# isaac-chandler/cuda-raytracer

Measured on AMD Instinct MI355X. Metric: Mrays/s (live ray segments/s, teapot), higher is better.
Workload: dtype f32

## Files before the change

### cuda-raytracer_amd/csrc/rt_render.hip

```cpp
#include "rt_common.h"

#include <algorithm>
#include <chrono>
#include <cstdio>
#include <cstdlib>
#include <cstring>
#include <string>
#include <thread>
#include <vector>

#include <rccl/rccl.h>

#pragma clang fp contract(off)

int rtamd_render_multi(const rt_scene *scene, const rt_opts *opts, float *fb_out, rt_stats *stats);

using namespace rtamd;

namespace {

#ifndef RT_INFLIGHT
#define RT_INFLIGHT 20
#endif
#ifndef RT_TRACE_OCC
// ... 50 lines not shown
    static FastDiv of(uint32_t d) {
        FastDiv f;
        if (d > 1) {
            f.l = 32 - __builtin_clz(d - 1);
            f.m = (uint32_t)((((uint64_t)1 << (31 + f.l)) + d - 1) / d);
        }
        return f;
    }
    __device__ __forceinline__ uint32_t div(uint32_t n) const { return l == 0 ? n : (__umulhi(n, m) >> (l - 1)); }
};

struct SlotMap {
    FastDiv by_stripe;
    uint32_t skip, base;
    static SlotMap identity() { return SlotMap{FastDiv::of(0x7fffffffu), 0u, 0u}; }
    static SlotMap of(uint32_t stripe, int count, int index) {
        return SlotMap{FastDiv::of(stripe), (uint32_t)(count - 1) * stripe, (uint32_t)index * stripe};
    }
    __device__ __forceinline__ uint32_t ray(uint32_t s) const { return s + by_stripe.div(s) * skip + base; }
};

template <int FIRST>
__device__ __forceinline__ uint32_t first_ray(const SlotMap &m, uint32_t slot) {
    return FIRST == 2 ? m.ray(slot) : slot;
}

struct PassArgs {
    int rtc;
    uint32_t gen_seed_term;
    FastDiv by_rtc, by_width;
    SlotMap map;
};

__device__ __forceinline__ V3 primary_dir(const DevScene &S, int i, const PassArgs &pa) {
    Rng rng = pcg_seed((uint32_t)i * 0x85810BEAu + pa.gen_seed_term);
    uint32_t z;
    asm volatile("v_mov_b32 %0, 0" : "=v"(z));
    rng.inc += z;
    const uint32_t pixel = pa.by_rtc.div((uint32_t)i);
    const uint32_t yy = pa.by_width.div(pixel);
    const int x = (int)(pixel - yy * (uint32_t)S.width), y = (int)yy;
    const float xc = (x + random01(rng)) * S.inv_w;
    const float yc = (y + random01(rng)) * S.inv_h;
    return normalise(S.tl + xc * S.sr - yc * S.su);
}

#ifndef RT_FUSED_MAX_TRIS
#define RT_FUSED_MAX_TRIS 4096
#endif
#ifndef RT_SORT_GRID
#define RT_SORT_GRID 0
#endif

template <bool SORTED, bool COUNT, int FIRST>
__global__ __launch_bounds__(kBlock) RT_TRACE_ATTR void trace_kernel(DevScene S, PassArgs pa, const float4 *__restrict__ geo,
                                                       const uint32_t *__restrict__ live_count,
                                                       uint32_t *__restrict__ queue, float2 *__restrict__ hits,
                                                       uint32_t *__restrict__ overflow, Counters *__restrict__ ctr,
                                                       unsigned long long *__restrict__ tspan) {
    __shared__ uint2 stack[(kStackLds + 1) * kBlock];
    const unsigned long long t_start = wall_clock64();
    uint2 *col = stack + threadIdx.x;
    const uint32_t lanes = gridDim.x * kBlock, gl = blockIdx.x * kBlock + threadIdx.x;
    const uint32_t dist_half = lanes * (kStackMax - kStackLds);
    const uint32_t L = __builtin_amdgcn_readfirstlane(*live_count);
    const uint32_t waves = gridDim.x * (kBlock / 64);
    const uint32_t chunk = min((uint32_t)kChunkMax, max((uint32_t)kChunkMin, (L / (4 * waves) + 63) & ~63u));
    uint32_t shard = blockIdx.x % kQueues, tried = 0;
    uint32_t q_next = 0, q_end = 0;
    bool exhausted = false;
    int slot = -1;
    V3 o{0, 0, 0}, d{0, 0, 0};
    float ix = 0, iy = 0, iz = 0, closest = 0;
    bool finite_inv = true;
    bool wave_nonfinite = false;
    int index = -1, sp = 0;
    uint32_t ref = 0;
    int ti = 0, te = 0;
    unsigned pn = 0, iv = 0, tt = 0, nlive = 0;
#ifdef RT_PROFILE
    unsigned long long prof[14] = {0, 0, 0, 0, 0, 0, 0, 0, 0, 0, 0, 0, 0, 0};
#endif
    auto node_step = [&](float4 a, float4 b, float4 c, uint2 kids) -> bool {
        if (COUNT) iv++;
        float t0, t1;
        bool h0, h1;
        slab_pair(a, b, c, o, ix, iy, iz, closest, h0, h1, t0, t1);
        if (__builtin_expect(wave_nonfinite, 0)) {
            float u0, u1;
            const bool g0 = slab(a.x, a.z, b.x, b.z, c.x, c.z, o, ix, iy, iz, closest, u0);
            const bool g1 = slab(a.y, a.w, b.y, b.w, c.y, c.w, o, ix, iy, iz, closest, u1);
            if (!finite_inv) { h0 = g0; h1 = g1; t0 = u0; t1 = u1; }
        }
        const bool both = h0 && h1, any = h0 || h1;
        const bool sel1 = h1 && (!h0 || t0 < t1);
        const uint32_t next_ref = sel1 ? kids.y : kids.x, near_ref = sel1 ? kids.x : kids.y;
        const float next_t = sel1 ? t1 : t0, near_t = sel1 ? t0 : t1;
        col[min(sp, kStackLds) * kBlock] = make_uint2(near_ref, __float_as_uint(near_t));
        if (__builtin_expect(both && sp >= kStackLds, 0)) {
            overflow[(sp - kStackLds) * lanes + gl] = near_ref;
            overflow[dist_half + (sp - kStackLds) * lanes + gl] = __float_as_uint(near_t);
        }
        if (both) sp++;
        ref = any ? next_ref : ref;
        const bool descend = any && !(next_t >= closest);
        bool need = !descend;
        if (descend) {
            if (COUNT) pn++;
            if (ref & kLeaf) {
                leaf_range(S, ref, ti, te);
                need = ti == te;
            }
        }
        return need;
    };
    auto pop_loop = [&](bool need) {
        while (need) {
            PROF(10, 1);
            const bool empty = sp == 0;
            sp = empty ? 0 : sp - 1;
            uint2 e = col[min(sp, kStackLds) * kBlock];
            asm volatile("" : "+v"(e.x), "+v"(e.y));
            if (__builtin_expect(__ballot(sp >= kStackLds) != 0, 0)) {
                if (sp >= kStackLds) {
                    e.x = overflow[(sp - kStackLds) * lanes + gl];
                    e.y = overflow[dist_half + (sp - kStackLds) * lanes + gl];
                }
            }
            const bool take = !empty && !(__uint_as_float(e.y) >= closest);
            slot = empty ? -2 - slot : slot;
            ref = take ? e.x : ref;
            if (COUNT) pn += take ? 1u : 0u;
            const bool leaf = take && (ref & kLeaf);
            if (__builtin_expect(leaf && (ref & kBigLeaf), 0)) {
                leaf_range(S, ref, ti, te);
            } else {
                ti = leaf ? (int)(ref & 0xFFFFFFu) : ti;
                te = leaf ? ti + (int)((ref >> 24) & 0x3Fu) : te;
            }
            need = !empty && (!take || (leaf && ti == te));
        }
    };
    const bool root_internal = !(S.root_ref & kLeaf);
    float4 ra{0, 0, 0, 0}, rb{0, 0, 0, 0}, rc{0, 0, 0, 0};
    uint2 rk{0, 0};
    if (root_internal) {
        const float4 *rr = S.nodes + (size_t)S.root_ref * 4;
        const float4 x0 = rr[0], x1 = rr[1], x2 = rr[2];
        const uint2 k = *reinterpret_cast<const uint2 *>(rr + 3);
#define RT_U(v) __int_as_float(__builtin_amdgcn_readfirstlane(__float_as_int(v)))
        ra = make_float4(RT_U(x0.x), RT_U(x0.y), RT_U(x0.z), RT_U(x0.w));
        rb = make_float4(RT_U(x1.x), RT_U(x1.y), RT_U(x1.z), RT_U(x1.w));
        rc = make_float4(RT_U(x2.x), RT_U(x2.y), RT_U(x2.z), RT_U(x2.w));
#undef RT_U
        rk = make_uint2(__builtin_amdgcn_readfirstlane(k.x), __builtin_amdgcn_readfirstlane(k.y));
    }
    while (true) {
        unsigned long long idle = __ballot(slot < 0);
        if (!exhausted && __popcll(idle) >= (FIRST ? kRefillFirst : kRefill)) {
            PROF(6, 1);
            if (slot <= -2) {
                hits[-2 - slot] = make_float2(closest, __int_as_float(index));
                slot = -1;
            }
            bool fresh = false;
            while (idle && !exhausted) {
                if (q_next >= q_end) {
                    const uint32_t seg_lo = (uint32_t)(((uint64_t)L * shard) / kQueues);
                    const uint32_t seg_hi = (uint32_t)(((uint64_t)L * (shard + 1)) / kQueues);
                    uint32_t c = 0;
                    if (lane_id() == 0) c = atomicAdd(queue + shard * kQueueStride, chunk);
                    c = __builtin_amdgcn_readfirstlane(__shfl(c, 0)) + seg_lo;
                    if (c >= seg_hi) {
                        shard = (shard + 1) % kQueues;
                        if (++tried == kQueues) exhausted = true;
                        continue;
                    }
                    q_next = c;
                    q_end = min(c + chunk, seg_hi);
                }
                const uint32_t avail = q_end - q_next;
                const uint32_t r = rank_below(idle);
                const bool take = slot < 0 && r < avail;
                const unsigned long long took = __ballot(take);
                if (take) { slot = (int)(q_next + r); fresh = true; }
                q_next += (uint32_t)__popcll(took);
                idle &= ~took;
            }
            if (fresh) {
                {
                    nlive++;
                    if (FIRST) {
                        o = S.cam;
                        d = primary_dir(S, (int)first_ray<FIRST>(pa.map, (uint32_t)slot), pa);
                    } else {
                        const float4 *rp = geo + (size_t)slot * 2;
                        const float4 r0 = rp[0];
                        const float2 r1 = *reinterpret_cast<const float2 *>(rp + 1);
                        o = v3(r0.x, r0.y, r0.z);
                        d = v3(r0.w, r1.x, r1.y);
                    }
                    ix = 1 / d.x; iy = 1 / d.y; iz = 1 / d.z;
                    finite_inv = __builtin_isfinite(ix) && __builtin_isfinite(iy) && __builtin_isfinite(iz);

                    closest = 1e30f;
                    index = -1;
                    for (int i = 0; i < S.sphere_count; i++) {
                        const float4 sph = S.spheres[i];
                        float t;
                        if (ray_sphere(o, d, v3(sph.x, sph.y, sph.z), sph.w, closest, t)) { closest = t; index = i; }
                    }
                    ref = S.root_ref;
                    sp = 0;
                    if (COUNT) pn++;
                    ti = te = 0;
                    if (ref & kLeaf) {
                        leaf_range(S, ref, ti, te);
                        if (ti == te) {
                            hits[slot] = make_float2(closest, __int_as_float(index));
                            slot = -1;
                        }
                    }
                }
            }
            wave_nonfinite = __ballot(slot >= 0 && !finite_inv) != 0;
            if (root_internal && __ballot(fresh && slot >= 0)) {
                bool need = false;
                if (fresh && slot >= 0) need = node_step(ra, rb, rc, rk);
                pop_loop(need);
            }
        }
        if (!__ballot(slot >= 0)) {
            if (exhausted) break;
            PROF(7, 1);
            continue;
        }
#ifdef RT_PROFILE
        {
            const unsigned long long act = __ballot(slot >= 0), lf = __ballot(slot >= 0 && ti < te);
            PROF(0, 1); PROF(1, __popcll(act)); PROF(2, __popcll(lf));
            PROF(3, lf != 0); PROF(4, (act & ~lf) != 0);
            const bool mixed = lf != 0 && (act & ~lf) != 0;
            PROF(8, mixed);
            if (mixed) PROF(9, min(__popcll(lf), __popcll(act & ~lf)));
            const uintptr_t ra = slot >= 0 ? (uintptr_t)(ti < te ? S.tris + (size_t)ti * 3 : S.nodes + (size_t)ref * 4) : 0;
            const int first = __builtin_ctzll(act);
            const uintptr_t r0 = ((uintptr_t)__shfl((unsigned)(ra >> 32), first) << 32) | __shfl((unsigned)ra, first);
            const unsigned long long same = __ballot(slot >= 0 && ra == r0);
            PROF(12, same == act);
            PROF(13, 4 * __popcll(same) >= 3 * __popcll(act));
        }
#endif
        if (slot < 0) continue;
        bool need = false;
        const bool in_leaf = ti < te;
        const float4 *rec = in_leaf ? S.tris + (size_t)ti * 3 : S.nodes + (size_t)ref * 4;
        const float4 a = rec[0], b = rec[1], c = rec[2];
        uint2 kids = make_uint2(0, 0);
        if (!in_leaf) kids = *reinterpret_cast<const uint2 *>(rec + 3);
        if (in_leaf) {
            const float4 q0 = a, q1 = b;
            const float q2 = c.x;
            if (COUNT) tt++;
            float t;
            const bool hit =
                ray_triangle_flat(o, d, v3(q0.x, q0.y, q0.z), v3(q0.w, q1.x, q1.y), v3(q1.z, q1.w, q2), closest, t);
            closest = hit ? t : closest;
            index = hit ? S.sphere_count + ti : index;
            need = ++ti == te;
        } else {
            need = node_step(a, b, c, kids);
        }
#ifdef RT_PROFILE
        if (__ballot(need)) PROF(5, 1);
#endif
        pop_loop(need);
    }
    if (slot <= -2) hits[-2 - slot] = make_float2(closest, __int_as_float(index));
    Counters *cs = ctr + ((blockIdx.x * (kBlock / 64) + (threadIdx.x >> 6)) & (kCtrSlots - 1));
    const unsigned long long nl = wave_sum(nlive);
    if (COUNT) {
        const unsigned long long a = wave_sum(pn), b = wave_sum(iv), t = wave_sum(tt);
        if (lane_id() == 0) {
            atomicAdd(&cs->pn, a);
            atomicAdd(&cs->iv, b);
            atomicAdd(&cs->tt, t);
            atomicAdd(&cs->st, nl * (unsigned long long)S.sphere_count);
        }
    }
    if (lane_id() == 0 && nl) atomicAdd(&cs->live, nl);
    if (tspan) {
        __syncthreads();
        if (threadIdx.x == 0) {
            atomicMin(&tspan[blockIdx.x % kSpanSlots], t_start);
            atomicMax(&tspan[kSpanSlots + blockIdx.x % kSpanSlots], (unsigned long long)wall_clock64());
        }
    }
#ifdef RT_PROFILE
    prof[11] = wave_sum((unsigned)prof[10]);
    if (lane_id() == 0)
        for (int i = 0; i < 14; i++)
            if (i != 10) atomicAdd(&g_prof[FIRST ? 0 : 1][i], prof[i]);
#endif
}

struct Shaded {
    V3 no, nd, T;
    V3 C;
    uint32_t ray;
    int kind;
    bool acc_holds;
};
struct ShadeIn {
    float2 h;
    uint32_t ray, seed;
    bool acc_holds;
    float4 r0, r1;
    float tz;
};
template <bool SORTED, int FIRST, bool INLINE>
__device__ __forceinline__ ShadeIn shade_in(const PassArgs &pa, int slot, const float4 *__restrict__ geo,
                                            const float *__restrict__ tz, const uint32_t *__restrict__ rid,
                                            const float2 *__restrict__ hits, const uint32_t *__restrict__ seed_of) {
    ShadeIn in{};
    const uint32_t ray0 = first_ray<FIRST>(pa.map, (uint32_t)slot);
    const uint32_t rv = FIRST ? (FIRST == 2 ? ray0 : (uint32_t)slot) : rid[slot];
    in.ray = rv & ~kAccFlag;
    in.acc_holds = (rv & kAccFlag) != 0;
    in.seed = (!FIRST && seed_of) ? seed_of[slot] : (SORTED || FIRST) ? (FIRST == 2 ? ray0 : (uint32_t)slot) : in.ray;
    if (!INLINE) in.h = hits[slot];
    if (!FIRST) {
        in.r0 = geo[(size_t)slot * 2];
        in.r1 = geo[(size_t)slot * 2 + 1];
        in.tz = tz[slot];
    }
// ... 590 lines not shown
}
__global__ __launch_bounds__(kBlock) void add4_kernel(float *__restrict__ img, const float *__restrict__ add, int n) {
    const int i = blockIdx.x * kBlock + threadIdx.x;
    const int n4 = n >> 2;
    if (i < n4) {
        float4 a = reinterpret_cast<float4 *>(img)[i];
        const float4 b = reinterpret_cast<const float4 *>(add)[i];
        a.x = a.x + b.x; a.y = a.y + b.y; a.z = a.z + b.z; a.w = a.w + b.w;
        reinterpret_cast<float4 *>(img)[i] = a;
    }
    if (i < (n & 3)) img[(n4 << 2) + i] = img[(n4 << 2) + i] + add[(n4 << 2) + i];
}

__attribute__((constructor(101))) void rtamd_default_hw_queues() {
    setenv("GPU_MAX_HW_QUEUES", "24", 0);
}
int queues_granted() {
    const char *q = std::getenv("GPU_MAX_HW_QUEUES");
    const int n = q ? std::atoi(q) : 0;
    return n > 0 ? n : 4;
}

}

int rtamd::trace_closest_blocks_per_cu(int &per_cu) {
    HIPCHK(hipOccupancyMaxActiveBlocksPerMultiprocessor(&per_cu, trace_kernel<false, false, 0>, kBlock, 0));
    return RT_OK;
}
void rtamd::launch_trace_closest(bool count, int grid, hipStream_t s, const DevScene &ds, const float4 *geo,
                                 const uint32_t *live, uint32_t *queue, float2 *hits, uint32_t *overflow, Counters *ctr) {
    const PassArgs pa{1, 0u, FastDiv::of(1), FastDiv::of((uint32_t)ds.width), SlotMap::identity()};
    if (count)
        hipLaunchKernelGGL((trace_kernel<false, true, 0>), dim3(grid), dim3(kBlock), 0, s, ds, pa, geo, live, queue, hits,
                           overflow, ctr, nullptr);
    else
        hipLaunchKernelGGL((trace_kernel<false, false, 0>), dim3(grid), dim3(kBlock), 0, s, ds, pa, geo, live, queue, hits,
                           overflow, ctr, nullptr);
}

struct InitTimer {
    std::chrono::high_resolution_clock::time_point t = std::chrono::high_resolution_clock::now();
    std::string out;
    bool on = std::getenv("RTAMD_TIMING") != nullptr;
    void mark(const char *what) {
        if (!on) return;
        const auto now = std::chrono::high_resolution_clock::now();
        char buf[96];
        std::snprintf(buf, sizeof(buf), " %s %.1f ms,", what, std::chrono::duration<double, std::milli>(now - t).count());
        out += buf;
        t = now;
    }
    void report() const { if (on) std::fprintf(stderr, "rt_renderer init:%s\n", out.c_str()); }
};

struct PassCtx {
    hipStream_t stream = nullptr;
    DevBuf<float4> geo[2], acc;
    DevBuf<float> tz[2];
    DevBuf<uint32_t> rid[2], sort_counts, sort_offsets, sort_totals, live, queue, overflow;
    DevBuf<uint8_t> bkt;
    DevBuf<float2> hits;
    DevBuf<uint32_t> home_of;
    DevBuf<float> psum;
    DevBuf<uint32_t> gslot[2], newpos, glive;
    DevBuf<uint8_t> gbytes, lbytes;
    uint32_t *lg_host = nullptr;
    hipEvent_t lg_ready = nullptr;
    int t_p = 0, t_k = 0, t_b = -1, t_rtc = 0, t_rem = 0, t_n = 0, t_cur = 0, t_tiles_g = 0;
    uint64_t t_lg = 0;
    hipEvent_t fb_done = nullptr;
// ... 5 lines not shown
        if (lg_host) (void)hipHostFree(lg_host);
        if (lg_ready) (void)hipEventDestroy(lg_ready);
        for (auto e : events) (void)hipEventDestroy(e);
        if (fb_done) (void)hipEventDestroy(fb_done);
        if (done) (void)hipEventDestroy(done);
        if (stream) (void)hipStreamDestroy(stream);
    }
    int open() {
        if (stream) return RT_OK;
        HIPCHK(hipStreamCreateWithFlags(&stream, hipStreamNonBlocking));
        HIPCHK(hipEventCreateWithFlags(&fb_done, hipEventDisableTiming));
        HIPCHK(hipEventCreateWithFlags(&done, hipEventDisableTiming));
        return RT_OK;
    }
    hipEvent_t event() {
        if (ev == events.size()) {
            hipEvent_t e;
            if (hipEventCreate(&e) != hipSuccess) return nullptr;
            events.push_back(e);
        }
        return events[ev++];
    }
};

struct rt_renderer {
    bool sort = true, counters = false;
    int tile_count = 1, tile_index = 0, tile_rows = 8;
    bool pass_events = true;
    bool fused = false;
    bool inline_hits = false;
    int fused_upto = -1;
    bool home = false;
    uint32_t home_base = 0;
    int width = 0, height = 0, spp = 0, bounces = 0;
    SceneDev scene;
    DevBuf<float> fb;
    DevBuf<unsigned long long> tspans;
    int wall_khz = 0;
    std::vector<double> launch_ms;
    std::vector<uint32_t> launch_live;
    bool shade_hist = !std::getenv("RTAMD_SHADE_HIST") || std::atoi(std::getenv("RTAMD_SHADE_HIST")) != 0;
    int stagger_us = std::getenv("RTAMD_STAGGER_US") ? std::max(0, std::min(20000, std::atoi(std::getenv("RTAMD_STAGGER_US"))))
                                                    : kStaggerUs;
    int short_stagger_us = std::getenv("RTAMD_STAGGER_SHORT_US")
                               ? std::max(0, std::min(20000, std::atoi(std::getenv("RTAMD_STAGGER_SHORT_US")))) : kStaggerShortUs;
    PassCtx ctx[kInflight];
    int pass_hint = 0;
    int inflight_limit = 0;
    int trace_blocks = 0;
    int trace_blocks_max = 0;
    int nctx = 1;
    int inflight_cap = kInflight;
    hipEvent_t t_begin = nullptr, t_end = nullptr;

    ~rt_renderer() {
        (void)hipSetDevice(scene.device);
        if (run_pending && t_end) (void)hipEventSynchronize(t_end);
        for (hipEvent_t e : pass_done) (void)hipEventDestroy(e);
        if (xcomm) {
            (void)hipSetDevice(scene.device);
            if (failed) (void)ncclCommAbort(static_cast<ncclComm_t>(xcomm));
            for (auto &c : ctx)
                if (c.stream) (void)hipStreamSynchronize(c.stream);
            if (!failed) (void)ncclCommDestroy(static_cast<ncclComm_t>(xcomm));
        }
        if (xhost) (void)hipHostFree(xhost);
// ... 40 lines not shown
        if (tsort()) {
            fused = false;
            fused_upto = -1;
            inline_hits = false;
        }
        width = sc->width;
        height = sc->height;
        spp = sc->ray_count;
        bounces = sc->bounces;
        InitTimer tm;
        HIPCHK(hipSetDevice(o->device));
        tm.mark("hipSetDevice");
        if (int rc0 = ctx[0].open()) return rc0;
        tm.mark("first stream");
        HIPCHK(hipEventCreate(&t_begin));
        HIPCHK(hipEventCreate(&t_end));
        hipStream_t s0 = stream();
        int rc;
        if ((rc = scene.init(sc, o->device, s0))) return rc;
        const int64_t pixels = (int64_t)width * height;
        const int64_t max_rays = pixels * std::min(20, std::max(1, spp));
        if (max_rays > 0x7fffffff / 3) return rtamd::fail(RT_E_INVALID, "image too large for 32-bit ray indices");
        if ((rc = fb.alloc((size_t)pixels * 3))) return rc;
        int per_cu = 0;
        tm.mark("scene upload");
        HIPCHK(hipOccupancyMaxActiveBlocksPerMultiprocessor(&per_cu, trace_kernel<true, false, false>, kBlock, 0));
        tm.mark("occupancy query");
        trace_blocks_max = std::max(1, scene.cus * std::max(1, per_cu));
        trace_blocks = trace_blocks_max;
        const int tiles = tile_stride(max_rays);
        home = sort && !tiled() && bounces >= 2 && (fused || fused_upto >= 0);
        if (const char *e = std::getenv("RTAMD_HOME")) home = home && std::atoi(e) != 0;
        home_base = (uint32_t)max_rays;
        const size_t ctx_bytes = (size_t)max_rays * (2 * (32 + 4 + 4) + 16 + 1 + 8 + (tsort() ? 2 * 4 + 4 + 2 : 0) +
                                                     (home ? 16 + 4 : 0)) +
                                 (size_t)trace_blocks_max * kBlock * 8 * (kStackMax - kStackLds) + ((size_t)1 << 20);
        size_t mem_free = 0, mem_total = 0;
        HIPCHK(hipMemGetInfo(&mem_free, &mem_total));
        size_t cap = kInflight;
        if (inflight_limit > 0) cap = std::min<size_t>(cap, (size_t)inflight_limit);
        if (const char *e = std::getenv("RTAMD_INFLIGHT")) cap = std::min<size_t>(cap, (size_t)std::max(1, std::atoi(e)));
        cap = std::min<size_t>(cap, (size_t)queues_granted());
        inflight_cap = (int)cap;
        if (pass_hint > 0) cap = std::min<size_t>(cap, (size_t)pass_hint);
        nctx = (int)std::min<size_t>({cap, (size_t)std::max(1, pass_count()),
                                                    std::max<size_t>(1, mem_free / 2 / ctx_bytes)});
        if (tsort() && (size_t)nctx < std::min<size_t>(cap, (size_t)std::max(1, pass_count())))
            return rtamd::fail(RT_E_OOM, "pixel tiles with sort on: device memory holds only " + std::to_string(nctx) +
                                             " passes in flight; set RTAMD_INFLIGHT to the same lower value on every owner");
        const int inflight = nctx;
        for (int k = 0; k < inflight; k++) {
            PassCtx &c = ctx[k];
            if ((rc = c.open())) return rc;
            for (int q = 0; q < 2; q++) {
                if ((rc = c.geo[q].alloc((size_t)max_rays * 2))) return rc;
                if ((rc = c.tz[q].alloc((size_t)max_rays))) return rc;
                if ((rc = c.rid[q].alloc((size_t)max_rays))) return rc;
            }
            if ((rc = c.bkt.alloc((size_t)max_rays))) return rc;
            if ((rc = c.acc.alloc((size_t)max_rays * (home ? 2 : 1)))) return rc;
            if (home && (rc = c.home_of.alloc((size_t)max_rays))) return rc;
            if ((rc = c.sort_counts.alloc((size_t)kBuckets * tiles))) return rc;
            if ((rc = c.sort_offsets.alloc((size_t)kBuckets * tiles))) return rc;
            if ((rc = c.sort_totals.alloc(kBuckets))) return rc;
            if ((rc = c.live.alloc((size_t)bounces + 1))) return rc;
            if ((rc = c.queue.alloc((size_t)(bounces + 1) * kQueues * kQueueStride))) return rc;
// ... 31 lines not shown
        const int sgrid = std::min(grid, scene.cus * RT_SHADE_BPC);
        const int sort_grid = std::max(1, std::min(max_tiles(n), RT_SORT_GRID > 0 ? RT_SORT_GRID : scene.cus * 8));
        hipStream_t st = c.stream;
        int cur = 0;
        if (n == 0) {
            for (int k = 0; pass_events && k < 3 * bounces + 2 * (bounces - 1); k++) {
                hipEvent_t e = c.event();
                if (!e) return rtamd::fail(RT_E_HIP, "hipEventCreate failed");
                HIPCHK(hipEventRecord(e, st));
            }
            HIPCHK(hipMemsetAsync(sums, 0, (size_t)pixels * 3 * sizeof(float), st));
            return RT_OK;
        }
        hipLaunchKernelGGL(fill_live_kernel, dim3(1), dim3(256), 0, st, c.live.p, (uint32_t)n, bounces + 1, c.queue.p, tspan);
        const uint32_t stripe_px = (uint32_t)(tile_rows * width);
        const SlotMap pix = tiled() ? SlotMap::of(stripe_px, tile_count, tile_index) : SlotMap::identity();
        const SlotMap map = tiled() ? SlotMap::of(stripe_px * (uint32_t)rtc, tile_count, tile_index) : SlotMap::identity();
        const PassArgs pa{rtc, 709579u * (uint32_t)remaining, FastDiv::of((uint32_t)rtc), FastDiv::of((uint32_t)width),
                          map};
        for (int b = 0; b < bounces; b++) {
            const uint32_t seed_term = 279220567u * (uint32_t)(remaining * 20 + b);
            hipEvent_t e0 = nullptr, em = nullptr, e1 = nullptr;
            if (pass_events) {
                e0 = c.event(); em = c.event(); e1 = c.event();
                if (!e0 || !em || !e1) return rtamd::fail(RT_E_HIP, "hipEventCreate failed");
                HIPCHK(hipEventRecord(e0, st));
            }
            const uint32_t *lv = c.live.p + b;
            uint32_t *q = c.queue.p + (size_t)b * kQueues * kQueueStride;
            const bool last = b + 1 == bounces;
            uint32_t *hist = shade_hist && !last ? c.sort_counts.p : nullptr;
#define RT_PROCESS3(SORTED, COUNT, FIRST)                                                                         \
    do {                                                                                                         \
        if (!inline_hits)                                                                                        \
            hipLaunchKernelGGL((trace_kernel<SORTED, COUNT, FIRST>), dim3(tgrid), dim3(kBlock), 0, st, scene.ds, pa, \
                               c.geo[cur].p, lv, q, c.hits.p, c.overflow.p, scene.ctr.p,                         \
                               tspan ? tspan + kSpanWords * b : nullptr);                                        \
        if (em) HIPCHK(hipEventRecord(em, st));                                                                  \
        if (inline_hits)                                                                                         \
            hipLaunchKernelGGL((shade_kernel<SORTED, COUNT, FIRST, true, true>), dim3(sgrid), dim3(kBlock), 0, st,\
                               scene.ds, pa, c.geo[cur].p, c.tz[cur].p, c.rid[cur].p, c.acc.p, c.bkt.p, lv, c.hits.p, \
                               seed_term, (int)last, scene.ctr.p, nullptr, hist, tiles, (int)(home && b == 0));  \
        else if (fused || b <= fused_upto)                                                                       \
            hipLaunchKernelGGL((shade_kernel<SORTED, COUNT, FIRST, true, false>), dim3(sgrid), dim3(kBlock), 0, \
                               st, scene.ds, pa, c.geo[cur].p, c.tz[cur].p, c.rid[cur].p, c.acc.p, c.bkt.p, lv, c.hits.p, \
                               seed_term, (int)last, scene.ctr.p, nullptr, hist, tiles, (int)(home && b == 0));  \
        else                                                                                                     \
            hipLaunchKernelGGL((shade_kernel<SORTED, COUNT, FIRST, false, false>), dim3(sgrid), dim3(kBlock), 0, \
                               st, scene.ds, pa, c.geo[cur].p, c.tz[cur].p, c.rid[cur].p, c.acc.p, c.bkt.p, lv, c.hits.p, \
                               seed_term, (int)last, scene.ctr.p, nullptr, hist, tiles, (int)(home && b == 0));  \
    } while (0)
#define RT_PROCESS(SORTED, COUNT)                                                                                \
    do {                                                                                                         \
        if (b == 0) RT_PROCESS3(SORTED, COUNT, 1); else RT_PROCESS3(SORTED, COUNT, 0);                           \
    } while (0)
            if (sort) {
                if (counters) RT_PROCESS(true, true); else RT_PROCESS(true, false);
            } else {
                if (b == 0 && tiled()) {
                    if (counters) RT_PROCESS3(false, true, 2); else RT_PROCESS3(false, false, 2);
                } else if (counters) RT_PROCESS(false, true); else RT_PROCESS(false, false);
            }
#undef RT_PROCESS
#undef RT_PROCESS3
            HIPCHK(hipGetLastError());
            if (pass_events) HIPCHK(hipEventRecord(e1, st));
            if (b + 1 != bounces) {
                hipEvent_t s0 = nullptr, s1 = nullptr;
                if (pass_events) {
                    s0 = c.event(); s1 = c.event();
// ... 76 lines not shown
        c.t_cur = 0;
        c.t_lg = (uint64_t)c.t_rtc * width * height;
        c.t_tiles_g = tile_stride((int64_t)c.t_lg);
        hipLaunchKernelGGL(fill_live_kernel, dim3(1), dim3(256), 0, c.stream, c.live.p, (uint32_t)c.t_n, bounces + 1,
                           c.queue.p, nullptr);
        hipLaunchKernelGGL(set_count_kernel, dim3(1), dim3(64), 0, c.stream, c.glive.p, (uint32_t)c.t_lg, nullptr);
        HIPCHK(hipGetLastError());
        return RT_OK;
    }
    PassArgs tsort_args(const PassCtx &c) const {
        const uint32_t stripe_px = (uint32_t)(tile_rows * width);
        return PassArgs{c.t_rtc, 709579u * (uint32_t)c.t_rem, FastDiv::of((uint32_t)c.t_rtc), FastDiv::of((uint32_t)width),
                        SlotMap::of(stripe_px * (uint32_t)c.t_rtc, tile_count, tile_index)};
    }
    int tsort_front(PassCtx &c, int b, int64_t &sorted) {
        hipStream_t st = c.stream;
        const PassArgs pa = tsort_args(c);
        const int grid = blocks_for(c.t_n);
        const int tgrid = std::max(1, std::min(grid, trace_blocks));
        const int sgrid = std::max(1, std::min(grid, scene.cus * RT_SHADE_BPC));
        const uint32_t seed_term = 279220567u * (uint32_t)(c.t_rem * 20 + b);
        const uint32_t *lv = c.live.p + b;
        uint32_t *q = c.queue.p + (size_t)b * kQueues * kQueueStride;
        const int last = b + 1 == bounces;
        const int cur = c.t_cur;
        if (!last) {
            const int zgrid = std::max(1, std::min(blocks_for((int64_t)(c.t_lg + 15) / 16), scene.cus * 8));
            hipLaunchKernelGGL(zero_bytes_kernel, dim3(zgrid), dim3(kBlock), 0, st, c.gbytes.p, c.lbytes.p, c.glive.p);
        }
        if (c.t_n == 0) return RT_OK;
#define RT_TS(COUNT)                                                                                           \
    do {                                                                                                           \
        if (b == 0) {                                                                                              \
            hipLaunchKernelGGL((trace_kernel<true, COUNT, 2>), dim3(tgrid), dim3(kBlock), 0, st, scene.ds, pa,           \
                               c.geo[cur].p, lv, q, c.hits.p, c.overflow.p, scene.ctr.p, nullptr);                       \
            hipLaunchKernelGGL((shade_kernel<true, COUNT, 2, false, false>), dim3(sgrid), dim3(kBlock), 0, st, scene.ds, \
                               pa, c.geo[cur].p, c.tz[cur].p, c.rid[cur].p, c.acc.p, c.bkt.p, lv, c.hits.p,         \
                               seed_term, last, scene.ctr.p, nullptr);                                                   \
        } else {                                                                                                   \
            hipLaunchKernelGGL((trace_kernel<true, COUNT, 0>), dim3(tgrid), dim3(kBlock), 0, st, scene.ds, pa,           \
                               c.geo[cur].p, lv, q, c.hits.p, c.overflow.p, scene.ctr.p, nullptr);                       \
            hipLaunchKernelGGL((shade_kernel<true, COUNT, 0, false, false>), dim3(sgrid), dim3(kBlock), 0, st, scene.ds, \
                               pa, c.geo[cur].p, c.tz[cur].p, c.rid[cur].p, c.acc.p, c.bkt.p, lv, c.hits.p,         \
                               seed_term, last, scene.ctr.p, c.gslot[cur].p);                                            \
        }                                                                                                          \
    } while (0)
        if (counters) RT_TS(true); else RT_TS(false);
#undef RT_TS
        if (!last) {
            if (b == 0)
                hipLaunchKernelGGL(tile_bytes_kernel<1>, dim3(sgrid), dim3(kBlock), 0, st, c.bkt.p, lv, c.gslot[cur].p,
                                   pa.map, c.gbytes.p, c.lbytes.p);
            else
                hipLaunchKernelGGL(tile_bytes_kernel<0>, dim3(sgrid), dim3(kBlock), 0, st, c.bkt.p, lv, c.gslot[cur].p,
                                   pa.map, c.gbytes.p, c.lbytes.p);
            sorted += c.t_n;
        }
        HIPCHK(hipGetLastError());
        return RT_OK;
    }
    int tsort_back(PassCtx &c, int b) {
        hipStream_t st = c.stream;
        const PassArgs pa = tsort_args(c);
        if (b > 0) {
            if (int rc = wait_event(c.lg_ready)) return rc;
            c.t_lg = *c.lg_host;
        }
        const uint64_t lg = c.t_lg;
        if (lg > 0) {
            int rc;
            if (x_on_device) {
                rc = xfn(xuser, c.gbytes.p, lg, st);
            } else {
                HIPCHK(hipMemcpyAsync(xhost, c.gbytes.p, lg, hipMemcpyDeviceToHost, st));
// ... 244 lines not shown
        run_sorted = sorted;
        run_generated = generated;
        run_w0 = w0;
        (void)async;
        return RT_OK;
    }
    int finish_run(rt_stats *st) {
        if (!run_pending) return rtamd::fail(RT_E_INVALID, "rt_renderer_finish: no run in flight");
        run_pending = false;
        HIPCHK(hipSetDevice(scene.device));
        const int count = run_count, inflight = run_inflight;
        const bool events = run_events, tsorted = run_tsort, inl = run_inline;
        const int64_t sorted = run_sorted, generated = run_generated;
        const auto w0 = run_w0;
        if (int rc = wait_event(t_end)) return rc;
        if (std::getenv("RTAMD_TIMING"))
            std::fprintf(stderr, "rt_renderer run: %d passes enqueued in %.2f ms (host), done at %.2f ms\n", count, run_enq_ms,
                         std::chrono::duration<double, std::milli>(std::chrono::high_resolution_clock::now() - w0).count());
#ifdef RT_PROFILE
        {
            unsigned long long pr[2][14];
            HIPCHK(hipMemcpyFromSymbol(pr, HIP_SYMBOL(g_prof), sizeof(pr)));
            for (int f = 0; f < 2; f++) {
                const unsigned long long *q = pr[f];
                const double it = (double)std::max(1ull, q[0]);
                std::fprintf(stderr, "RT_PROFILE %s wave_iters %llu active/iter %.2f leaf/iter %.2f iters_with_leaf %.3f "
                             "iters_with_inner %.3f iters_with_pop %.3f refills/iter %.3f idle_iters %llu mixed %.3f "
                             "minority/mixed %.2f lane_pops/iter %.3f uniform_record %.3f three_quarters_same %.3f\n",
                             f ? "later" : "bounce0", q[0], q[1] / it, q[2] / it, q[3] / it, q[4] / it, q[5] / it,
                             q[6] / it, q[7], q[8] / it, q[9] / (double)std::max(1ull, q[8]), q[11] / it, q[12] / it, q[13] / it);
            }
            std::memset(pr, 0, sizeof(pr));
            HIPCHK(hipMemcpyToSymbol(HIP_SYMBOL(g_prof), pr, sizeof(pr)));
        }
#endif
        if (st) {
            std::memset(st, 0, sizeof(*st));
            Counters c{};
            if (int rc = scene.read_counters(c)) return rc;
            float ms = 0;
            HIPCHK(hipEventElapsedTime(&ms, t_begin, t_end));
            st->kernel_ms = ms;
            double proc = 0, srt = 0, trc = 0;
            uint64_t trace_launches = 0;
            for (int q = 0; events && !tsorted && q < inflight; q++) {
                const int passes_here = count > q ? (count - q + inflight - 1) / inflight : 0;
                size_t e = 0;
                for (int r = 0; r < passes_here; r++)
                    for (int b = 0; b < bounces; b++) {
                        HIPCHK(hipEventElapsedTime(&ms, ctx[q].events[e], ctx[q].events[e + 2]));
                        proc += ms;
                        e += 3;
                        if (b + 1 != bounces) {
                            HIPCHK(hipEventElapsedTime(&ms, ctx[q].events[e], ctx[q].events[e + 1]));
                            srt += ms;
                            e += 2;
                        }
                    }
            }
            launch_ms.clear();
            launch_live.clear();
            if (events && !inl && !tsorted && count > 0 && run_span_words <= tspans.n) {
                std::vector<unsigned long long> sp(run_span_words);
                HIPCHK(hipMemcpy(sp.data(), tspans.p, sp.size() * sizeof(unsigned long long), hipMemcpyDeviceToHost));
                for (int k = 0; k < count; k++)
                    for (int b = 0; b < bounces; b++) {
// ... 279 lines not shown
    HIPCHK(hipSetDevice(r->scene.device));
    ncclUniqueId uid;
    std::memcpy(&uid, id, sizeof(uid));
    ncclComm_t comm = nullptr;
    const ncclResult_t e = ncclCommInitRank(&comm, nranks, uid, rank);
    if (e != ncclSuccess) return rtamd::fail(RT_E_HIP, std::string("Error ncclCommInitRank ") + ncclGetErrorString(e));
    r->xcomm = comm;
    return rt_renderer_set_exchange(r, rccl_exchange, comm, 1);
}

int rtamd_renderer_set_poll(rt_renderer *r, int (*fn)(void *), void *user) {
    if (!r) return rtamd::fail(RT_E_INVALID, "null renderer");
    r->xpoll = fn;
    r->xpoll_user = user;
    return RT_OK;
}

int rt_renderer_set_accumulate(rt_renderer *r, int32_t enable) {
    if (!r) return rtamd::fail(RT_E_INVALID, "null renderer");
    if (int rc = r->busy("rt_renderer_set_accumulate")) return rc;
    r->accumulate = enable != 0;
    return RT_OK;
}

int rt_renderer_set_counters(rt_renderer *r, int32_t enable) {
    if (!r) return rtamd::fail(RT_E_INVALID, "null renderer");
    if (int rc = r->busy("rt_renderer_set_counters")) return rc;
    r->counters = enable != 0;
    return RT_OK;
}

void rt_renderer_destroy(rt_renderer *r) { delete r; }

int rt_render(const rt_scene *scene, const rt_opts *opts, float *fb_out, rt_stats *stats) {
    using clk = std::chrono::high_resolution_clock;
    const auto w0 = clk::now();
    auto ms_since = [](clk::time_point t) { return std::chrono::duration<double, std::milli>(clk::now() - t).count(); };
    if (!fb_out) return rtamd::fail(RT_E_INVALID, "null framebuffer");
    rt_opts o;
    if (opts) o = *opts; else rt_default_opts(&o);
    if (o.device_count >= 1) {
        const int rc = check_scene(scene);
        return rc ? rc : rtamd_render_multi(scene, &o, fb_out, stats);
    }
    rt_renderer *r = nullptr;
    const int P = (scene->ray_count + 19) / 20;
    const int stride = std::max(1, o.pass_stride);
    const int hint = o.pass_count >= 0 ? o.pass_count : std::max(0, (P - o.pass_begin + stride - 1) / stride);
    int rc = create_renderer(scene, &o, &r, std::max(1, hint));
    if (rc) return rc;
    const char *ev = std::getenv("RTAMD_EVENTS");
    r->pass_events = ev && std::atoi(ev) != 0;
    const double t_create = ms_since(w0);
    auto w1 = clk::now();
    rc = r->run(o.pass_begin, o.pass_count, o.pass_stride, nullptr, stats);
    const double t_run = ms_since(w1);
    w1 = clk::now();
    if (!rc) rc = rt_renderer_read_framebuffer(r, fb_out);
    const double t_read = ms_since(w1);
    w1 = clk::now();
    const int inflight = r->nctx;
    delete r;
    const double t_free = ms_since(w1);
    if (std::getenv("RTAMD_TIMING"))
        std::fprintf(stderr, "rt_render: create %.1f ms (%d passes in flight), run %.1f ms, read %.1f ms, destroy %.1f ms\n",
                     t_create, inflight, t_run, t_read, t_free);
// ... 29 lines not shown
```

Baseline: 13700.

## Seed primary-ray traversal with each pixel's previously hit triangle

Adds a per-pixel table recording the triangle hit by an earlier primary ray, written only when traversal took many wave steps. A later primary ray for the same pixel first intersects that triangle and uses a slightly padded hit distance as its initial closest bound, so the BVH walk can prune more nodes. If the seeded traversal finds nothing, the ray is restarted without a seed so results stay correct. The cost is an extra triangle test and table read or write per primary ray, a second full traversal whenever the seed's bound rejects everything, and extra register pressure and branches in the seeded kernel variant.

```diff
diff --git a/cuda-raytracer_amd/csrc/rt_render.hip b/cuda-raytracer_amd/csrc/rt_render.hip
--- a/cuda-raytracer_amd/csrc/rt_render.hip
+++ b/cuda-raytracer_amd/csrc/rt_render.hip
@@ -106,6 +106,23 @@
     SlotMap map;
 };
 
+#ifndef RT_SEED_MIN_STEPS
+#define RT_SEED_MIN_STEPS 64
+#endif
+constexpr uint32_t kNoSeed = 0xFFFFFFFFu;
+constexpr uint32_t kSeedMinSteps = RT_SEED_MIN_STEPS;
+constexpr float kSeedGuard = 1e-4f;
+struct SeedArgs {
+    uint32_t *table;
+    uint32_t tris;
+#ifdef RTAMD_TEST_HOOKS
+    float bound_scale;
+#endif
+};
+#ifdef RT_PROFILE
+__device__ unsigned long long g_seed_prof[3];
+#endif
+
 __device__ __forceinline__ V3 primary_dir(const DevScene &S, int i, const PassArgs &pa) {
     Rng rng = pcg_seed((uint32_t)i * 0x85810BEAu + pa.gen_seed_term);
     uint32_t z;
@@ -126,17 +143,24 @@
 #define RT_SORT_GRID 0
 #endif
 
-template <bool SORTED, bool COUNT, int FIRST>
+template <bool SORTED, bool COUNT, int FIRST, bool SEED = false>
 __global__ __launch_bounds__(kBlock) RT_TRACE_ATTR void trace_kernel(DevScene S, PassArgs pa, const float4 *__restrict__ geo,
                                                        const uint32_t *__restrict__ live_count,
                                                        uint32_t *__restrict__ queue, float2 *__restrict__ hits,
                                                        uint32_t *__restrict__ overflow, Counters *__restrict__ ctr,
-                                                       unsigned long long *__restrict__ tspan) {
+                                                       unsigned long long *__restrict__ tspan, SeedArgs sd) {
+    constexpr bool SEEDED = SEED && FIRST != 0 && !COUNT;
     __shared__ uint2 stack[(kStackLds + 1) * kBlock];
     const unsigned long long t_start = wall_clock64();
     uint2 *col = stack + threadIdx.x;
     const uint32_t lanes = gridDim.x * kBlock, gl = blockIdx.x * kBlock + threadIdx.x;
     const uint32_t dist_half = lanes * (kStackMax - kStackLds);
+    auto lane_gl = [&]() -> uint32_t {
+        if (!SEEDED) return gl;
+        uint32_t ca = (uint32_t)(uintptr_t)col;
+        asm volatile("" : "+v"(ca));
+        return blockIdx.x * kBlock + (ca - (uint32_t)(uintptr_t)stack) / (uint32_t)sizeof(uint2);
+    };
     const uint32_t L = __builtin_amdgcn_readfirstlane(*live_count);
     const uint32_t waves = gridDim.x * (kBlock / 64);
     const uint32_t chunk = min((uint32_t)kChunkMax, max((uint32_t)kChunkMin, (L / (4 * waves) + 63) & ~63u));
@@ -146,7 +170,13 @@
     int slot = -1;
     V3 o{0, 0, 0}, d{0, 0, 0};
     float ix = 0, iy = 0, iz = 0, closest = 0;
+    uint32_t wsteps = 0;
+    uint32_t nlive_s = 0;
+#ifdef RT_PROFILE
+    unsigned sprof[3] = {0, 0, 0};
+#endif
     bool finite_inv = true;
+#define RT_LANE_FINITE (SEEDED ? __builtin_isfinite(ix) && __builtin_isfinite(iy) && __builtin_isfinite(iz) : finite_inv)
     bool wave_nonfinite = false;
     int index = -1, sp = 0;
     uint32_t ref = 0;
@@ -164,7 +194,7 @@
             float u0, u1;
             const bool g0 = slab(a.x, a.z, b.x, b.z, c.x, c.z, o, ix, iy, iz, closest, u0);
             const bool g1 = slab(a.y, a.w, b.y, b.w, c.y, c.w, o, ix, iy, iz, closest, u1);
-            if (!finite_inv) { h0 = g0; h1 = g1; t0 = u0; t1 = u1; }
+            if (!RT_LANE_FINITE) { h0 = g0; h1 = g1; t0 = u0; t1 = u1; }
         }
         const bool both = h0 && h1, any = h0 || h1;
         const bool sel1 = h1 && (!h0 || t0 < t1);
@@ -172,8 +202,9 @@
         const float next_t = sel1 ? t1 : t0, near_t = sel1 ? t0 : t1;
         col[min(sp, kStackLds) * kBlock] = make_uint2(near_ref, __float_as_uint(near_t));
         if (__builtin_expect(both && sp >= kStackLds, 0)) {
-            overflow[(sp - kStackLds) * lanes + gl] = near_ref;
-            overflow[dist_half + (sp - kStackLds) * lanes + gl] = __float_as_uint(near_t);
+            const uint32_t g = lane_gl();
+            overflow[(sp - kStackLds) * lanes + g] = near_ref;
+            overflow[dist_half + (sp - kStackLds) * lanes + g] = __float_as_uint(near_t);
         }
         if (both) sp++;
         ref = any ? next_ref : ref;
@@ -197,8 +228,9 @@
             asm volatile("" : "+v"(e.x), "+v"(e.y));
             if (__builtin_expect(__ballot(sp >= kStackLds) != 0, 0)) {
                 if (sp >= kStackLds) {
-                    e.x = overflow[(sp - kStackLds) * lanes + gl];
-                    e.y = overflow[dist_half + (sp - kStackLds) * lanes + gl];
+                    const uint32_t g = lane_gl();
+                    e.x = overflow[(sp - kStackLds) * lanes + g];
+                    e.y = overflow[dist_half + (sp - kStackLds) * lanes + g];
                 }
             }
             const bool take = !empty && !(__uint_as_float(e.y) >= closest);
@@ -231,13 +263,33 @@
     }
     while (true) {
         unsigned long long idle = __ballot(slot < 0);
-        if (!exhausted && __popcll(idle) >= (FIRST ? kRefillFirst : kRefill)) {
+        if ((!exhausted && __popcll(idle) >= (FIRST ? kRefillFirst : kRefill)) || (SEEDED && idle == ~0ull)) {
             PROF(6, 1);
+            bool fresh = false, again = false;
+            if (SEEDED) {
+                again = slot <= -2 && index == -1 && closest != 1e30f;
+                if (again) {
+                    slot = -2 - slot;
+                    fresh = true;
+#ifdef RT_PROFILE
+                    sprof[1]++;
+#endif
+                }
+                idle &= ~__ballot(again);
+            }
             if (slot <= -2) {
                 hits[-2 - slot] = make_float2(closest, __int_as_float(index));
+                if (SEEDED) {
+                    const uint32_t tri = (uint32_t)(index - S.sphere_count);
+                    if (sd.table && wsteps >= kSeedMinSteps && index >= S.sphere_count && tri < sd.tris) {
+                        sd.table[pa.by_rtc.div(first_ray<FIRST>(pa.map, (uint32_t)(-2 - slot)))] = tri;
+#ifdef RT_PROFILE
+                        sprof[2]++;
+#endif
+                    }
+                }
                 slot = -1;
             }
-            bool fresh = false;
             while (idle && !exhausted) {
                 if (q_next >= q_end) {
                     const uint32_t seg_lo = (uint32_t)(((uint64_t)L * shard) / kQueues);
@@ -261,21 +313,28 @@
                 q_next += (uint32_t)__popcll(took);
                 idle &= ~took;
             }
+            if (SEEDED) nlive_s += (uint32_t)__popcll(__ballot(fresh && !again));
+            if (SEEDED && __ballot(fresh && !again)) wsteps = 0;
             if (fresh) {
                 {
-                    nlive++;
-                    if (FIRST) {
-                        o = S.cam;
-                        d = primary_dir(S, (int)first_ray<FIRST>(pa.map, (uint32_t)slot), pa);
-                    } else {
-                        const float4 *rp = geo + (size_t)slot * 2;
-                        const float4 r0 = rp[0];
-                        const float2 r1 = *reinterpret_cast<const float2 *>(rp + 1);
-                        o = v3(r0.x, r0.y, r0.z);
-                        d = v3(r0.w, r1.x, r1.y);
+                    uint32_t seed = kNoSeed;
+                    if (!again) {
+                        if (!SEEDED) nlive++;
+                        if (FIRST) {
+                            const uint32_t ray = first_ray<FIRST>(pa.map, (uint32_t)slot);
+                            if (SEEDED) seed = sd.table ? sd.table[pa.by_rtc.div(ray)] : kNoSeed;
+                            o = S.cam;
+                            d = primary_dir(S, (int)ray, pa);
+                        } else {
+                            const float4 *rp = geo + (size_t)slot * 2;
+                            const float4 r0 = rp[0];
+                            const float2 r1 = *reinterpret_cast<const float2 *>(rp + 1);
+                            o = v3(r0.x, r0.y, r0.z);
+                            d = v3(r0.w, r1.x, r1.y);
+                        }
+                        ix = 1 / d.x; iy = 1 / d.y; iz = 1 / d.z;
+                        if (!SEEDED) finite_inv = __builtin_isfinite(ix) && __builtin_isfinite(iy) && __builtin_isfinite(iz);
                     }
-                    ix = 1 / d.x; iy = 1 / d.y; iz = 1 / d.z;
-                    finite_inv = __builtin_isfinite(ix) && __builtin_isfinite(iy) && __builtin_isfinite(iz);
 
                     closest = 1e30f;
                     index = -1;
@@ -283,6 +342,28 @@
                         const float4 sph = S.spheres[i];
                         float t;
                         if (ray_sphere(o, d, v3(sph.x, sph.y, sph.z), sph.w, closest, t)) { closest = t; index = i; }
+                    }
+                    if (SEEDED) {
+                        if (!again && seed < sd.tris) {
+                            const float4 *tp = S.tris + (size_t)seed * 3;
+                            const float4 q0 = tp[0], q1 = tp[1];
+                            const float q2 = tp[2].x;
+                            float ts;
+                            if (ray_triangle_flat(o, d, v3(q0.x, q0.y, q0.z), v3(q0.w, q1.x, q1.y), v3(q1.z, q1.w, q2), 1e30f,
+                                                  ts)) {
+                                float c0 = ts * (1.0f + kSeedGuard);
+#ifdef RTAMD_TEST_HOOKS
+                                c0 *= sd.bound_scale;
+#endif
+                                if (c0 < closest) {
+                                    closest = c0;
+                                    index = -1;
+#ifdef RT_PROFILE
+                                    sprof[0]++;
+#endif
+                                }
+                            }
+                        }
                     }
                     ref = S.root_ref;
                     sp = 0;
@@ -297,7 +378,7 @@
                     }
                 }
             }
-            wave_nonfinite = __ballot(slot >= 0 && !finite_inv) != 0;
+            wave_nonfinite = __ballot(slot >= 0 && !RT_LANE_FINITE) != 0;
             if (root_internal && __ballot(fresh && slot >= 0)) {
                 bool need = false;
                 if (fresh && slot >= 0) need = node_step(ra, rb, rc, rk);
@@ -305,10 +386,11 @@
             }
         }
         if (!__ballot(slot >= 0)) {
-            if (exhausted) break;
+            if (exhausted && !(SEEDED && __ballot(slot <= -2))) break;
             PROF(7, 1);
             continue;
         }
+        if (SEEDED) wsteps++;
 #ifdef RT_PROFILE
         {
             const unsigned long long act = __ballot(slot >= 0), lf = __ballot(slot >= 0 && ti < te);
@@ -350,9 +432,9 @@
 #endif
         pop_loop(need);
     }
-    if (slot <= -2) hits[-2 - slot] = make_float2(closest, __int_as_float(index));
+    if (!SEEDED && slot <= -2) hits[-2 - slot] = make_float2(closest, __int_as_float(index));
     Counters *cs = ctr + ((blockIdx.x * (kBlock / 64) + (threadIdx.x >> 6)) & (kCtrSlots - 1));
-    const unsigned long long nl = wave_sum(nlive);
+    const unsigned long long nl = SEEDED ? nlive_s : wave_sum(nlive);
     if (COUNT) {
         const unsigned long long a = wave_sum(pn), b = wave_sum(iv), t = wave_sum(tt);
         if (lane_id() == 0) {
@@ -362,6 +444,7 @@
             atomicAdd(&cs->st, nl * (unsigned long long)S.sphere_count);
         }
     }
+#undef RT_LANE_FINITE
     if (lane_id() == 0 && nl) atomicAdd(&cs->live, nl);
     if (tspan) {
         __syncthreads();
@@ -375,6 +458,11 @@
     if (lane_id() == 0)
         for (int i = 0; i < 14; i++)
             if (i != 10) atomicAdd(&g_prof[FIRST ? 0 : 1][i], prof[i]);
+    if (SEEDED)
+        for (int i = 0; i < 3; i++) {
+            const unsigned long long v = wave_sum(sprof[i]);
+            if (lane_id() == 0) atomicAdd(&g_seed_prof[i], v);
+        }
 #endif
 }
 
@@ -1031,10 +1119,10 @@
     const PassArgs pa{1, 0u, FastDiv::of(1), FastDiv::of((uint32_t)ds.width), SlotMap::identity()};
     if (count)
         hipLaunchKernelGGL((trace_kernel<false, true, 0>), dim3(grid), dim3(kBlock), 0, s, ds, pa, geo, live, queue, hits,
-                           overflow, ctr, nullptr);
+                           overflow, ctr, nullptr, SeedArgs{});
     else
         hipLaunchKernelGGL((trace_kernel<false, false, 0>), dim3(grid), dim3(kBlock), 0, s, ds, pa, geo, live, queue, hits,
-                           overflow, ctr, nullptr);
+                           overflow, ctr, nullptr, SeedArgs{});
 }
 
 struct InitTimer {
@@ -1106,6 +1194,15 @@
     int fused_upto = -1;
     bool home = false;
     uint32_t home_base = 0;
+    bool seed_on = false;
+    DevBuf<uint32_t> seeds;
+    uint32_t seed_tris = 0;
+#ifdef RTAMD_TEST_HOOKS
+    float seed_bound_scale = 1.f;
+    SeedArgs seed_args() const { return SeedArgs{seed_on ? seeds.p : nullptr, seed_tris, seed_bound_scale}; }
+#else
+    SeedArgs seed_args() const { return SeedArgs{seed_on ? seeds.p : nullptr, seed_tris}; }
+#endif
     int width = 0, height = 0, spp = 0, bounces = 0;
     SceneDev scene;
     DevBuf<float> fb;
@@ -1212,6 +1309,13 @@
         home = sort && !tiled() && bounces >= 2 && (fused || fused_upto >= 0);
         if (const char *e = std::getenv("RTAMD_HOME")) home = home && std::atoi(e) != 0;
         home_base = (uint32_t)max_rays;
+        seed_on = sc->triangle_count > 0;
+        if (const char *e = std::getenv("RTAMD_SEED")) seed_on = seed_on && std::atoi(e) != 0;
+        seed_tris = (uint32_t)sc->triangle_count;
+        if (seed_on) {
+            if ((rc = seeds.alloc((size_t)pixels))) return rc;
+            HIPCHK(hipMemsetAsync(seeds.p, 0xFF, (size_t)pixels * sizeof(uint32_t), s0));
+        }
         const size_t ctx_bytes = (size_t)max_rays * (2 * (32 + 4 + 4) + 16 + 1 + 8 + (tsort() ? 2 * 4 + 4 + 2 : 0) +
                                                      (home ? 16 + 4 : 0)) +
                                  (size_t)trace_blocks_max * kBlock * 8 * (kStackMax - kStackLds) + ((size_t)1 << 20);
@@ -1309,10 +1413,14 @@
             uint32_t *hist = shade_hist && !last ? c.sort_counts.p : nullptr;
 #define RT_PROCESS3(SORTED, COUNT, FIRST)                                                                         \
     do {                                                                                                         \
-        if (!inline_hits)                                                                                        \
+        if (!inline_hits && seed_on)                                                                             \
+            hipLaunchKernelGGL((trace_kernel<SORTED, COUNT, FIRST, ((FIRST) != 0 && !(COUNT))>), dim3(tgrid),    \
+                               dim3(kBlock), 0, st, scene.ds, pa, c.geo[cur].p, lv, q, c.hits.p, c.overflow.p,   \
+                               scene.ctr.p, tspan ? tspan + kSpanWords * b : nullptr, seed_args());              \
+        else if (!inline_hits)                                                                                   \
             hipLaunchKernelGGL((trace_kernel<SORTED, COUNT, FIRST>), dim3(tgrid), dim3(kBlock), 0, st, scene.ds, pa, \
                                c.geo[cur].p, lv, q, c.hits.p, c.overflow.p, scene.ctr.p,                         \
-                               tspan ? tspan + kSpanWords * b : nullptr);                                        \
+                               tspan ? tspan + kSpanWords * b : nullptr, SeedArgs{});                            \
         if (em) HIPCHK(hipEventRecord(em, st));                                                                  \
         if (inline_hits)                                                                                         \
             hipLaunchKernelGGL((shade_kernel<SORTED, COUNT, FIRST, true, true>), dim3(sgrid), dim3(kBlock), 0, st,\
@@ -1455,14 +1563,18 @@
 #define RT_TS(COUNT)                                                                                           \
     do {                                                                                                           \
         if (b == 0) {                                                                                              \
-            hipLaunchKernelGGL((trace_kernel<true, COUNT, 2>), dim3(tgrid), dim3(kBlock), 0, st, scene.ds, pa,           \
-                               c.geo[cur].p, lv, q, c.hits.p, c.overflow.p, scene.ctr.p, nullptr);                       \
+            if (seed_on)                                                                                           \
+                hipLaunchKernelGGL((trace_kernel<true, COUNT, 2, !(COUNT)>), dim3(tgrid), dim3(kBlock), 0, st, scene.ds, \
+                                   pa, c.geo[cur].p, lv, q, c.hits.p, c.overflow.p, scene.ctr.p, nullptr, seed_args()); \
+            else                                                                                                   \
+                hipLaunchKernelGGL((trace_kernel<true, COUNT, 2>), dim3(tgrid), dim3(kBlock), 0, st, scene.ds, pa,       \
+                                   c.geo[cur].p, lv, q, c.hits.p, c.overflow.p, scene.ctr.p, nullptr, SeedArgs{});       \
             hipLaunchKernelGGL((shade_kernel<true, COUNT, 2, false, false>), dim3(sgrid), dim3(kBlock), 0, st, scene.ds, \
                                pa, c.geo[cur].p, c.tz[cur].p, c.rid[cur].p, c.acc.p, c.bkt.p, lv, c.hits.p,         \
                                seed_term, last, scene.ctr.p, nullptr);                                                   \
         } else {                                                                                                   \
             hipLaunchKernelGGL((trace_kernel<true, COUNT, 0>), dim3(tgrid), dim3(kBlock), 0, st, scene.ds, pa,           \
-                               c.geo[cur].p, lv, q, c.hits.p, c.overflow.p, scene.ctr.p, nullptr);                       \
+                               c.geo[cur].p, lv, q, c.hits.p, c.overflow.p, scene.ctr.p, nullptr, SeedArgs{});           \
             hipLaunchKernelGGL((shade_kernel<true, COUNT, 0, false, false>), dim3(sgrid), dim3(kBlock), 0, st, scene.ds, \
                                pa, c.geo[cur].p, c.tz[cur].p, c.rid[cur].p, c.acc.p, c.bkt.p, lv, c.hits.p,         \
                                seed_term, last, scene.ctr.p, c.gslot[cur].p);                                            \
@@ -1773,6 +1885,12 @@
             }
             std::memset(pr, 0, sizeof(pr));
             HIPCHK(hipMemcpyToSymbol(HIP_SYMBOL(g_prof), pr, sizeof(pr)));
+            unsigned long long sp3[3];
+            HIPCHK(hipMemcpyFromSymbol(sp3, HIP_SYMBOL(g_seed_prof), sizeof(sp3)));
+            std::fprintf(stderr, "RT_PROFILE seed: primary rays seeded %llu, restarted unseeded %llu, table stores %llu\n",
+                         sp3[0], sp3[1], sp3[2]);
+            std::memset(sp3, 0, sizeof(sp3));
+            HIPCHK(hipMemcpyToSymbol(HIP_SYMBOL(g_seed_prof), sp3, sizeof(sp3)));
         }
 #endif
         if (st) {
@@ -2118,6 +2236,32 @@
 
 void rt_renderer_destroy(rt_renderer *r) { delete r; }
 
+#ifdef RTAMD_TEST_HOOKS
+int rt_test_seed_table_write(rt_renderer *r, const uint32_t *values, uint64_t n) {
+    if (!r || !values) return rtamd::fail(RT_E_INVALID, "null argument");
+    if (int rc = r->busy("rt_test_seed_table_write")) return rc;
+    if (!r->seed_on || n != r->seeds.n) return rtamd::fail(RT_E_INVALID, "seed table: off, or not width * height values");
+    HIPCHK(hipSetDevice(r->scene.device));
+    HIPCHK(hipMemcpy(r->seeds.p, values, n * sizeof(uint32_t), hipMemcpyHostToDevice));
+    return RT_OK;
+}
+int rt_test_seed_bound_scale(rt_renderer *r, float scale) {
+    if (!r) return rtamd::fail(RT_E_INVALID, "null renderer");
+    if (int rc = r->busy("rt_test_seed_bound_scale")) return rc;
+    r->seed_bound_scale = scale;
+    return RT_OK;
+}
+int rt_test_seed_table_read(rt_renderer *r, uint32_t *values, uint64_t n) {
+    if (!r || !values) return rtamd::fail(RT_E_INVALID, "null argument");
+    if (int rc = r->busy("rt_test_seed_table_read")) return rc;
+    if (!r->seed_on || n != r->seeds.n) return rtamd::fail(RT_E_INVALID, "seed table: off, or not width * height values");
+    HIPCHK(hipSetDevice(r->scene.device));
+    HIPCHK(hipDeviceSynchronize());
+    HIPCHK(hipMemcpy(values, r->seeds.p, n * sizeof(uint32_t), hipMemcpyDeviceToHost));
+    return RT_OK;
+}
+#endif
+
 int rt_render(const rt_scene *scene, const rt_opts *opts, float *fb_out, rt_stats *stats) {
     using clk = std::chrono::high_resolution_clock;
     const auto w0 = clk::now();
```

Result: faster. 13840, median of 6 (+1.0%).
